# POSTECH-CVLab/SCNeRF

Measured on AMD Instinct MI355X. Metric: rays/sec (64+128 samples/ray) train-step, higher is better.
Workload: dtype f32 (3 x fp16 MFMA products per product, fp32 accumulate); 1 GPU; configs[1]: 4096 rays x (64 coarse + 128 fine), coarse+fine NeRF (D=8, W=256), fwd+bwd of render_rays per GPU, perturb=1, raw_noise_std=1; precomputed rays of a fixed camera; rays_per_gpu=4096, parallelism=ray-parallel x1, no collective at N = 1

## Files before the change

include/scnerf_hip.h:

```cpp
#ifndef SCNERF_HIP_H
#define SCNERF_HIP_H

#include <stdint.h>

#ifdef __cplusplus
extern "C" {
#endif

#define SCNERF_ABI_VERSION 4

int scnerf_abi_version(void);


int scnerf_searchsorted(const float* a, const float* v, int64_t* out, int nrow, int nrow_a,
                        int nrow_v, int na, int nv, int side_left, void* stream);

int scnerf_sample_pdf(const float* bins, const float* weights, const float* u, int u_row_stride,
                      float* samples, int64_t* inds, float* cdf, int n, int nb, int ns,
                      void* stream);

int scnerf_render_randoms(unsigned long long seed, unsigned long long call, float* t_rand, long long n_t_rand,
                          float* u, long long n_u, float* noise_c, long long n_noise_c, float* noise_f,
                          long long n_noise_f, float raw_noise_std, void* stream);

// ... 327 lines not shown

int scnerf_ray_expand(const int* slot_of, long long n, long long n_live, int s_tot, int s_fine, const float* rgb_l,
                      const float* disp_l, const float* acc_l, const float* depth_l, const float* z_std_l, const float* raw_l,
                      const float* z_vals_l, const float* z_samples_l, const float* rgb0, const float* disp0,
                      const float* acc0, const float* depth0, float* rgb_map, float* disp_map, float* acc_map,
                      float* depth_map, float* z_std, float* raw, float* z_vals, float* z_samples, void* stream);


long long scnerf_live_compact_workspace_ints(long long n_samples);
int scnerf_live_compact(const float* d_raw, long long n_samples, int* workspace, int* live_idx, unsigned* xoff,
                        float* d_raw_live, int* n_live_dev, int* n_live_host, void* stream);
int scnerf_live_gather(const int* live_idx, long long n_live, long long n_samples, const unsigned* masks, const float* pts,
                       int pt_dims, const float* viewdirs, int vd_stride, int samples_per_ray, unsigned* masks_live,
                       float* pts_live, float* vd_live, void* stream);
int scnerf_live_scatter_rows(const float* src, const int* live_idx, float* dst, long long n_live, int w, long long n,
                             void* stream);
int scnerf_live_remap_maxima(const int* live_idx, long long n_live, const float* amax_src, int n_chunks_src,
                             long long chunk_src, float* amax_dst, int n_chunks_dst, long long chunk_dst, int rows, void* stream);
int scnerf_mlp_bwd_h3_masks(int pt_dims, const float* d_raw, const float* pts, const float* viewdirs, int vd_stride,
                            int samples_per_ray, const float* wpacked_bwd, const short* stream_bwd, const float* scales,
                            const unsigned* masks, float* grads, float* d_pts, float* d_views, long long n_samples,
                            float* chunk_amax, int n_chunks, long long chunk_samples, int* guard_flags, int* guard_any,
                            float* guard_report, int lean, void* stream);
int scnerf_nerf_wgrad_h3_live(int pt_dims, const float* save, long long n_samples_src, int n_chunks_src,
                              const float* grads_live, const float* d_raw, const int* live_idx, const unsigned* xoff,
                              long long n_live, int n_chunks_live, float* workspace, float* flat_grad, int accumulate,
                              const float* amax_x_live, const float* amax_z_live, const float* scales, const float* flat_params,
                              void* ev_before, void* ev_after, void* stream);


long long scnerf_occ_compact_workspace_ints(long long n_samples);
int scnerf_occ_compact(const float* pts, long long n_samples, const float* viewdirs, int vd_stride, int samples_per_ray,
                       const int* bits, int R, float lo_x, float lo_y, float lo_z, float inv_x, float inv_y, float inv_z,
                       int* workspace, int* live_idx, int* slot_of, float* pts_live, float* vd_live, int* n_live_dev,
                       int* n_live_host, void* stream);
int scnerf_occ_expand_raw(const float* raw_live, const int* slot_of, float* raw, long long n_samples, long long n_live,
                          void* stream);
int scnerf_occ_probe_points(long long first_cell, long long n_cells, int R, int k, float lo_x, float lo_y, float lo_z,
                            float cell_x, float cell_y, float cell_z, float off0, float off1, float off2, float* pts,
                            void* stream);
int scnerf_occ_accumulate(const float* raw, float sigma_min, long long first_cell, long long n_cells, int R, int k, int* bits,
                          void* stream);
int scnerf_occ_dilate(const int* bits_in, int* bits_out, int R, void* stream);

long long scnerf_occ_compact4_workspace_ints(long long n_samples);
int scnerf_occ_compact4(const float* pts, long long n_samples, const float* viewdirs, int vd_stride, int samples_per_ray,
// ... 24 lines not shown
```

scnerf_amd/_capi.py:

```python
from __future__ import annotations

import ctypes
import os
from ctypes import c_int, c_longlong, c_void_p, c_float, c_double

D = c_double

F = c_float

_HERE = os.path.dirname(os.path.abspath(__file__))
LIB_PATH = os.environ.get("SCNERF_HIP_LIB") or os.path.join(_HERE, "libscnerf_hip.so")

P = c_void_p
I = c_int
LL = c_longlong

PROTOTYPES = {
    "scnerf_abi_version": [],
    "scnerf_searchsorted": [P, P, P, I, I, I, I, I, I, P],
    "scnerf_sample_pdf": [P, P, P, I, P, P, P, I, I, I, P],
    "scnerf_render_randoms": [ctypes.c_ulonglong, ctypes.c_ulonglong, P, LL, P, LL, P, LL, P, LL, F, P],
    "scnerf_coarse_sample": [P, I, P, P, P, P, I, I, I, P],
    "scnerf_fine_sample": [P, I, P, P, P, I, P, P, P, P, P, P, I, I, I, P],
    "scnerf_camera_rays_fwd": [P, P, I, P, I, P, P, F, I, P, P, F, I, P, F, P, F, I, I, I, I, P, P, I, P],
# ... 62 lines not shown
    "scnerf_nerf_wgrad_h3": [I, P, P, P, LL, I, P, P, I, P, P, P, P, P, P],
    "scnerf_wgrad256_half": [P, P, LL, I, P, P, P, P, P, P],
    "scnerf_wgrad_half_narrow": [P, I, P, I, I, I, LL, I, P, P, P, P, P, I, LL, P],
    "scnerf_mlp_fwd_h3_lean": [I, P, P, I, I, P, P, P, P, P, LL, P, I, LL, P, P, P, I, P],
    "scnerf_mlp_bwd_h3_lean": [I, P, P, P, I, I, P, P, P, P, P, P, P, LL, P, I, LL, P, P, P, I, P],
    "scnerf_coarse_stage_fwd_h3_lean": [P, I, P, P, I, P, P, P, P, P, I, P, P, P, P, P, P, P, P, I, I, P, I, LL,
                                        P, P, P, I, P],
    "scnerf_fine_stage_fwd_h3_lean": [P, I, P, P, P, I, P, P, P, P, P, I, P, P, P, P, P, P, P, P, P, P, P, P, I, I, I, P,
                                      I, LL, P, P, P, I, P],
    "scnerf_nerf_wgrad_h3_lean": [I, P, P, P, LL, I, P, P, I, P, P, P, P, P, P, P],
    "scnerf_wgrad_lean_finish": [P, P, P, P, I, P],
    "scnerf_wgrad_lean_finish_pd": [I, P, P, P, P, I, P],
    "scnerf_image_metrics": [P, LL, LL, LL, LL, P, LL, LL, LL, LL, I, I, I, I, P, I, F, F, F, I, P, P, P, P, P],
    "scnerf_ray_batch": [I, ctypes.c_ulonglong, ctypes.c_ulonglong, P, I, I, I, LL, LL, P, I, I, LL, LL, LL, LL, LL, I, I, I,
                         P, P, P, P, P],
    "scnerf_ray_compact": [P, F, P, P, P, P, LL, P],
    "scnerf_ray_rows_gather": [P, P, P, LL, I, LL, P],
    "scnerf_ray_expand": [P, LL, LL, I, I] + [P] * 8 + [P] * 4 + [P] * 8 + [P],
    "scnerf_live_compact": [P, LL, P, P, P, P, P, P, P],
    "scnerf_live_gather": [P, LL, LL, P, P, I, P, I, I, P, P, P, P],
    "scnerf_live_remap_maxima": [P, LL, P, I, LL, P, I, LL, I, P],
    "scnerf_live_scatter_rows": [P, P, P, LL, I, LL, P],
    "scnerf_mlp_bwd_h3_masks": [I, P, P, P, I, I, P, P, P, P, P, P, P, LL, P, I, LL, P, P, P, I, P],
    "scnerf_nerf_wgrad_h3_live": [I, P, LL, I, P, P, P, P, LL, I, P, P, I, P, P, P, P, P, P, P],
    "scnerf_occ_compact": [P, LL, P, I, I, P, I, F, F, F, F, F, F, P, P, P, P, P, P, P, P],
    "scnerf_occ_expand_raw": [P, P, P, LL, LL, P],
    "scnerf_occ_probe_points": [LL, LL, I, I, F, F, F, F, F, F, F, F, F, P, P],
    "scnerf_occ_accumulate": [P, F, LL, LL, I, I, P, P],
    "scnerf_occ_dilate": [P, P, I, P],
    "scnerf_occ_compact4": [P, LL, P, I, I, P, I, F, F, F, F, F, F, P, P, P, P, P, P, P, P],
    "scnerf_occ_probe_points_inverted": [LL, LL, I, I, F, F, F, F, F, F, F, F, F, P, P],
    "scnerf_seg_compact": [P, LL, I, I, I, P, P, I, P, I, F, F, F, F, F, F, P, P, P, P, P, P, P, P],
    "scnerf_seg_expand_raw": [P, P, P, LL, I, I, I, LL, P],
    "scnerf_seg_transmittance": [P, P, P, I, LL, I, I, I, I, I, D, P, P, P, P],
}


SIZE_FUNCS = {"scnerf_mlp_save_floats": [I, LL], "scnerf_mlp_grad_floats": [LL],
              "scnerf_wgrad_workspace_floats": [I, I, I],
              "scnerf_nerf_wgrad_workspace_floats": [I],
              "scnerf_h3_scale_floats": [],
              "scnerf_wgrad_chunk_samples": [LL, I],
              "scnerf_camera_bwd_workspace_floats": [I],
              "scnerf_live_compact_workspace_ints": [LL],
              "scnerf_occ_compact_workspace_ints": [LL],
              "scnerf_occ_compact4_workspace_ints": [LL],
# ... 50 lines not shown
```

scnerf_amd/csrc/mlp_bwd_h3.hip:

```cpp
#include <cstdint>

#include <scn_wave.h>

#include "launch.h"
#include "mlp_bwd_h3_api.h"
#include "mlp_common.h"
#include "scnerf_hip.h"

extern "C" int scnerf_mlp_bwd_h3_lean(int pt_dims, const float* d_raw, const float* pts, const float* viewdirs,
                                      int vd_stride, int samples_per_ray, const float* wpacked_bwd, const short* stream_bwd,
                                      const float* scales, const float* save, float* grads, float* d_pts, float* d_views,
                                      long long n_samples, float* chunk_amax, int n_chunks, long long chunk_samples,
                                      int* guard_flags, int* guard_any, float* guard_report, int lean, void* stream) {
    SCN_RETURN_IF(!d_raw || !pts || !viewdirs || !wpacked_bwd || !stream_bwd || !scales || !save || !grads, SCN_EINVAL);
    SCN_RETURN_IF(!d_pts != !d_views, SCN_EINVAL);
    SCN_RETURN_IF(samples_per_ray < 1 || vd_stride < 3 || n_samples < 0 || (pt_dims != 3 && pt_dims != 4), SCN_EINVAL);
    SCN_RETURN_IF(n_samples >= (1LL << 31), SCN_ENOSUP);
    SCN_RETURN_IF(chunk_amax && (n_chunks < 1 || chunk_samples < 32 || chunk_samples % 32), SCN_EINVAL);
    SCN_RETURN_IF(!guard_flags != !guard_any || (guard_report && !guard_flags), SCN_EINVAL);
    if (n_samples == 0) return 0;
    hipStream_t st = (hipStream_t)stream;
    const scn::h3b::ChunkMaxima cm{chunk_amax, n_chunks, lean != 0, (long)chunk_samples, {guard_flags, guard_any, guard_report}};
    return pt_dims == 3 ? scn::h3b::bwd_h3_pd3(d_raw, pts, viewdirs, vd_stride, samples_per_ray, wpacked_bwd, stream_bwd, scales, save, grads, d_pts, d_views, n_samples, cm, st)
                        : scn::h3b::bwd_h3_pd4(d_raw, pts, viewdirs, vd_stride, samples_per_ray, wpacked_bwd, stream_bwd, scales, save, grads, d_pts, d_views, n_samples, cm, st);
}

extern "C" int scnerf_mlp_bwd_h3_masks(int pt_dims, const float* d_raw, const float* pts, const float* viewdirs,
                                       int vd_stride, int samples_per_ray, const float* wpacked_bwd, const short* stream_bwd,
                                       const float* scales, const unsigned* masks, float* grads, float* d_pts, float* d_views,
                                       long long n_samples, float* chunk_amax, int n_chunks, long long chunk_samples,
                                       int* guard_flags, int* guard_any, float* guard_report, int lean, void* stream) {
    SCN_RETURN_IF(!masks || n_samples < 0 || (pt_dims != 3 && pt_dims != 4), SCN_EINVAL);
    const long long per_sample = pt_dims == 3 ? scn::mlp::Var<3>::kSavePerSample : scn::mlp::Var<4>::kSavePerSample;
    const uintptr_t base = reinterpret_cast<uintptr_t>(masks) - (uintptr_t)(per_sample * scn::mlp::padded_samples((long)n_samples)) * sizeof(float);
    return scnerf_mlp_bwd_h3_lean(pt_dims, d_raw, pts, viewdirs, vd_stride, samples_per_ray, wpacked_bwd, stream_bwd, scales,
                                  reinterpret_cast<const float*>(base), grads, d_pts, d_views, n_samples, chunk_amax, n_chunks,
                                  chunk_samples, guard_flags, guard_any, guard_report, lean, stream);
}

extern "C" int scnerf_mlp_bwd_h3_guarded(int pt_dims, const float* d_raw, const float* pts, const float* viewdirs,
                                         int vd_stride, int samples_per_ray, const float* wpacked_bwd, const short* stream_bwd,
                                         const float* scales, const float* save, float* grads, float* d_pts, float* d_views,
                                         long long n_samples, float* chunk_amax, int n_chunks, long long chunk_samples,
                                         int* guard_flags, int* guard_any, float* guard_report, void* stream) {
    return scnerf_mlp_bwd_h3_lean(pt_dims, d_raw, pts, viewdirs, vd_stride, samples_per_ray, wpacked_bwd, stream_bwd, scales, save,
                                  grads, d_pts, d_views, n_samples, chunk_amax, n_chunks, chunk_samples, guard_flags, guard_any,
                                  guard_report, 0, stream);
}

extern "C" int scnerf_mlp_bwd_h3(int pt_dims, const float* d_raw, const float* pts, const float* viewdirs, int vd_stride,
                                 int samples_per_ray, const float* wpacked_bwd, const short* stream_bwd, const float* scales,
                                 const float* save, float* grads, float* d_pts, float* d_views, long long n_samples,
                                 float* chunk_amax, int n_chunks, long long chunk_samples, void* stream) {
    return scnerf_mlp_bwd_h3_guarded(pt_dims, d_raw, pts, viewdirs, vd_stride, samples_per_ray, wpacked_bwd, stream_bwd, scales,
                                     save, grads, d_pts, d_views, n_samples, chunk_amax, n_chunks, chunk_samples, nullptr,
                                     nullptr, nullptr, stream);
}
```

scnerf_amd/csrc/mlp_bwd_h3_api.h:

```cpp
#pragma once
#include <hip/hip_runtime.h>

#include "resident_guard.h"

namespace scn {
namespace h3b {

struct ChunkMaxima { float* amax; int n_chunks; int lean; long chunk; ResidentGuard guard; };

int bwd_h3_pd3(const float* d_raw, const float* pts, const float* viewdirs, int vd_stride, int samples_per_ray,
               const float* wpacked_bwd, const short* stream_bwd, const float* scales, const float* save, float* grads,
               float* d_pts, float* d_views, long long n_samples, ChunkMaxima cm, hipStream_t st);
int bwd_h3_pd4(const float* d_raw, const float* pts, const float* viewdirs, int vd_stride, int samples_per_ray,
               const float* wpacked_bwd, const short* stream_bwd, const float* scales, const float* save, float* grads,
               float* d_pts, float* d_views, long long n_samples, ChunkMaxima cm, hipStream_t st);

}
}
```

scnerf_amd/csrc/mlp_bwd_h3_kernel.h:

```cpp
#pragma once
#include <scn_wave.h>

#include "launch.h"
#include "mlp_bwd_h3_api.h"
#include "mlp_h3.h"

namespace scn {
namespace h3b {

using namespace scn::mlp;
using namespace scn::h3;


template <int PD, int L, int NS>
__device__ __forceinline__ void pe_backward(float x, float y, float z, float w, int h, const float (&de)[NS], float* d_a, float* d_b) {
    const float a = h ? y : x;
    float freq = 1.f;
    if constexpr (PD == 3) {
        float ga = de[3 * L];
        float gz = h ? 0.f : de[3 * L + 1];
#pragma unroll
        for (int f = 0; f < L; ++f) {
            float s0, c0, s1, c1;
            sincos(a * freq, &s0, &c0);
// ... 76 lines not shown
            ol[sl][c0] = pack_f16(residual_f16<0>(v[0], s_next, hp), residual_f16<1>(v[1], s_next, hp));
        } else if constexpr (SUB == 8) {
            hp = pack_f16_scaled(v[2], v[3], s_next);
        } else if constexpr (SUB == 9) {
            oh[sl][c0 + 1] = hp;
            ol[sl][c0 + 1] = pack_f16(residual_f16<0>(v[2], s_next, hp), residual_f16<1>(v[3], s_next, hp));
        } else if constexpr (SUB == 10) {
            if constexpr (lab::kNoStore) {
            } else if constexpr (KIND == 2) {
                store_written_through_window(uniform_global_rw(save + (4 * T + q) * 1024), pinned_here(lane16), f32x4{v[0], v[1], v[2], v[3]}, this->window);
            } else {
                store_written_through_at(uniform_global_rw(save + (4 * T + q) * 1024), pinned_here(lane16), f32x4{v[0], v[1], v[2], v[3]});
            }
        }
    }
};


template <int PD>
__host__ __device__ constexpr unsigned bwd_lds_bytes() {
    return (unsigned)(kStreamLds + 256 * 4 + Var<PD>::kES * kThreads * 4);
}

template <int PD, bool IG>
__global__ __launch_bounds__(kThreads, 1) void mlp_bwd_h3_kernel(
    const float* __restrict__ d_raw, const float* __restrict__ pts, const float* __restrict__ viewdirs, int vd_stride,
    int samples_per_ray, const float* __restrict__ wbk, const short* __restrict__ wh3, const float* __restrict__ sc,
    const float* __restrict__ save, float* __restrict__ grads, float* __restrict__ d_pts, float* __restrict__ d_views, long P,
    ChunkMaxima cm) {
    using V = Var<PD>;
    constexpr int ES = V::kES, ET = V::kET;
    claim_whole_register_file();
    const int lane = lane_id();
    const int m = lane & 31, h = lane >> 5;
    const long wave_tile = (long)blockIdx.x * 4 + uniform(wave_id());
    const long p = wave_tile * kSamplesPerWave + m;
    const bool live = p < P;
    const long pc = live ? p : P - 1;
    const long Ppad = padded_samples(P);

    Wave w;
    w.lds = dynamic_lds<char>();
    w.tid16 = threadIdx.x * 16u;
    w.lane16 = (unsigned)lane * 16u;
    float* const alpha_tab = reinterpret_cast<float*>(w.lds + kStreamLds);
    f32x4* const park = reinterpret_cast<f32x4*>(w.lds + kStreamLds + 256 * 4) + threadIdx.x;
    stream_prime(w.ws, wh3, w.lds, w.tid16);
    alpha_tab[threadIdx.x] = wbk[V::kBwdAlphaW + threadIdx.x];

    f32x4 dr = *reinterpret_cast<const f32x4*>(d_raw + pc * 4);
    if (!live) dr = f32x4{0.f, 0.f, 0.f, 0.f};
    const float dsigma = dr[3];

    u32x4 bh[2][16], bl[2][16];
    f32x16 acc[2][2];
    auto section = [&](int offset, int width) {
        return uniform_global_rw(grads + (long)offset * Ppad + wave_tile * (32L * width));
    };
    auto load_gate = [&](int sect) {
        const unsigned* base = reinterpret_cast<const unsigned*>(save + (long)V::kSavePerSample * Ppad);
        return load_at<u32x4>(uniform_global(base + ((long)sect * (Ppad / 32) + wave_tile) * 256), w.lane16);
    };
    auto scale_of = [&](int layer, int what) { return sc[layer * kScaleStride + what]; };
    auto amax_of = [&](float a) { return fmaxf(a, shfl_xor(a, 32)); };
    const int chunk_of_tile = cm.amax ? uniform((int)((unsigned)(wave_tile * kSamplesPerWave) / (unsigned)cm.chunk)) : 0;
    auto note_chunk_max = [&](int job, float v) __attribute__((always_inline)) {
        if (cm.amax == nullptr) return;
        v = fmaxf(v, shfl_xor(v, 16)); v = fmaxf(v, shfl_xor(v, 8)); v = fmaxf(v, shfl_xor(v, 4));
        v = fmaxf(v, shfl_xor(v, 2)); v = fmaxf(v, shfl_xor(v, 1));
        if (lane_id() == 0) atomic_max_nonneg(cm.amax + (long)job * cm.n_chunks + chunk_of_tile, v);
    };
    auto guard = [&](int guard_layer, float am, float s) __attribute__((always_inline)) {
        guard_check(cm.guard, guard_layer, am, s, live, wave_tile);
    };
    using GateEpi = BwdEpi<0>;
    auto make_gate = [&](int layer, float s_in, int mask_sect, int out_offset, int out_width) {
        GateEpi e;
        e.os = inv_pow2(s_in) * scale_of(layer, kSwInv);
        e.s_next = 1.f;
        e.am = 0.f;
        e.save = section(out_offset, out_width);
        e.lane16 = w.lane16;
        e.gate = load_gate(mask_sect);
        return e;
// ... 7 lines not shown
        cut8(x8, s_rgb, rh, rl);
    }
    GateEpi epiv = make_gate(kLayerRgb, s_rgb, 8, kGradDzv, 128);
    epiv.s_next = scale_for(scale_of(kLayerRgb, kBoundAT) * am_rgb);
    block_sync();
    ring_prime(w);
    {
        auto operand = [&](auto, u32x4& xh, u32x4& xl) { xh = rh; xl = rl; };
        tile_pair<0, 1>(w, acc[0], operand, NoFill{});
        tile_pair<1, 1>(w, acc[1], operand, NoFill{});
        epi_all<GateEpi, 0>(epiv, acc[0], bh[1], bl[1]);
        epi_all<GateEpi, 1>(epiv, acc[1], bh[1], bl[1]);
    }
    const float am_v = amax_of(epiv.am);
    note_chunk_max(8, am_v);
    guard(kLayerViews, am_v, epiv.s_next);

    auto hv_operand = [&](auto s_tag, u32x4& xh, u32x4& xl) {
        constexpr int s = decltype(s_tag)::value;
        xh = bh[1][s]; xl = bl[1][s];
    };
    if constexpr (!IG) {
        skip_units<2, 4>(w, NoFill{});
        const long ray = (long)((unsigned)pc / (unsigned)samples_per_ray);
        note_chunk_max(11, fmaxf(fmaxf(1.f, fabsf(viewdirs[ray * vd_stride + 0])),
                                 fmaxf(fabsf(viewdirs[ray * vd_stride + 1]), fabsf(viewdirs[ray * vd_stride + 2]))));
    } else {
        f32x16 acce[2];
        tile_single<2, 4>(w, acce, hv_operand, NoFill{});
        const float os = inv_pow2(epiv.s_next) * scale_of(kLayerViews, kSwInv);
        float dev[16];
#pragma unroll
        for (int r = 0; r < 16; ++r) dev[r] = (acce[0][r] + acce[1][r]) * os;
        const long ray = (long)((unsigned)pc / (unsigned)samples_per_ray);
        note_chunk_max(11, fmaxf(fmaxf(1.f, fabsf(viewdirs[ray * vd_stride + 0])),
                                 fmaxf(fabsf(viewdirs[ray * vd_stride + 1]), fabsf(viewdirs[ray * vd_stride + 2]))));
        float gxy, gz;
        pe_backward<3, 4, 16>(viewdirs[ray * vd_stride + 0], viewdirs[ray * vd_stride + 1], viewdirs[ray * vd_stride + 2], 0.f, h, dev, &gxy, &gz);
        const float oxy = shfl_xor(gxy, 32), oz = shfl_xor(gz, 32);
        if (live && h == 0) {
            d_views[p * 3 + 0] = gxy;
            d_views[p * 3 + 1] = oxy;
            d_views[p * 3 + 2] = gz + oz;
        }
    }
    using LinEpi = BwdEpi<2>;
    LinEpi epif;
    epif.os = inv_pow2(epiv.s_next) * scale_of(kLayerViews, kSwInv);
    epif.s_next = scale_for(scale_of(kLayerViews, kBoundAT) * am_v);
    epif.am = 0.f;
    epif.save = section(kGradDfeat, 256);
    epif.lane16 = w.lane16;
    epif.window = cm.lean ? kStoreWindowShut : kStoreWindowOpen;
    tile_pair<6, 8>(w, acc[0], hv_operand, NoFill{});
    tile_pair<14, 8>(w, acc[1], hv_operand, [&](auto sg) { epi_slot<LinEpi, 0, decltype(sg)::value, 6>(epif, acc[0], bh[0], bl[0]); });
    tile_pair<22, 8>(w, acc[0], hv_operand, [&](auto sg) { epi_slot<LinEpi, 1, decltype(sg)::value, 6>(epif, acc[1], bh[0], bl[0]); });
    tile_pair<30, 8>(w, acc[1], hv_operand, [&](auto sg) { epi_slot<LinEpi, 2, decltype(sg)::value, 6>(epif, acc[0], bh[0], bl[0]); });

    auto trunk_layer = [&](auto x_tag, auto& pend, auto& cur, float bound_a, float bound_extra, int job)
                           __attribute__((always_inline)) {
        constexpr int X = decltype(x_tag)::value;
        auto operand = [&](auto s_tag, u32x4& xh, u32x4& xl) {
            constexpr int s = decltype(s_tag)::value;
            xh = bh[X][s]; xl = bl[X][s];
        };
        using Pend = std::remove_reference_t<decltype(pend)>;
// ... 56 lines not shown
        const float am5 = amax_of(prev.am);
        note_chunk_max(4, am5);
        guard(5, am5, prev.s_next);
        cur.s_next = scale_for(scale_of(5, kBoundAT) * am5);
        constexpr int U0 = 6;
        tile_pair<U0, 16>(w, acc[0], operand, NoFill{});
        tile_pair<U0 + 16, 16>(w, acc[1], operand, [&](auto sg) { epi_slot<GateEpi, 0, decltype(sg)::value, 12>(cur, acc[0], bh[0], bl[0]); });
        tile_pair<U0 + 32, 16>(w, acc[0], operand, [&](auto sg) { epi_slot<GateEpi, 1, decltype(sg)::value, 12>(cur, acc[1], bh[0], bl[0]); });
        tile_pair<U0 + 48, 16>(w, acc[1], operand, [&](auto sg) { epi_slot<GateEpi, 2, decltype(sg)::value, 12>(cur, acc[0], bh[0], bl[0]); });
        prev = cur;
    }
#pragma unroll 1
    for (int l = 4; l >= 2; l -= 2) {
        GateEpi cur = make_gate(l, prev.s_next, l - 1, kGradDz + (l - 1) * 256, 256);
        trunk_layer(I<0>{}, prev, cur, scale_of(l, kBoundAT), 0.f, l - 1);
        GateEpi cur2 = make_gate(l - 1, cur.s_next, l - 2, kGradDz + (l - 2) * 256, 256);
        trunk_layer(I<1>{}, cur, cur2, scale_of(l - 1, kBoundAT), 0.f, l - 2);
        prev = cur2;
    }
    if constexpr (!IG) {
        epi_all<GateEpi, 3>(prev, acc[1], bh[0], bl[0]);
        note_chunk_max(9, amax_of(prev.am));
        guard(0, amax_of(prev.am), prev.s_next);
        float am_e = fmaxf(fmaxf(1.f, fabsf(pts[pc * PD + 0])), fmaxf(fabsf(pts[pc * PD + 1]), fabsf(pts[pc * PD + 2])));
        if constexpr (PD == 4) am_e = fmaxf(am_e, fabsf(pts[pc * PD + 3]));
        note_chunk_max(10, am_e);
    } else {
        auto operand = [&](auto s_tag, u32x4& xh, u32x4& xl) {
            constexpr int s = decltype(s_tag)::value;
            xh = bh[0][s]; xl = bl[0][s];
        };
        float de[ES];
        tile_pair<6, 16>(w, acc[0], operand, [&](auto sg) { epi_slot<GateEpi, 3, decltype(sg)::value, 9>(prev, acc[1], bh[0], bl[0]); });
        const float os0 = inv_pow2(prev.s_next) * scale_of(0, kSwInv);
        note_chunk_max(9, amax_of(prev.am));
        guard(0, amax_of(prev.am), prev.s_next);
        auto add_pair = [&](auto t0_tag, f32x16 (&a)[2]) {
            constexpr int T0 = decltype(t0_tag)::value;
#pragma unroll
            for (int x = 0; x < 2; ++x)
                if (16 * (T0 + x) < ES) {
#pragma unroll
                    for (int q = 0; q < 4; ++q) {
                        const f32x4 pk = park[(4 * (T0 + x) + q) * kThreads];
#pragma unroll
                        for (int j = 0; j < 4; ++j) de[16 * (T0 + x) + 4 * q + j] = __builtin_fmaf(a[x][4 * q + j], os0, pk[j]);
                    }
                }
        };
        add_pair(I<0>{}, acc[0]);
        if constexpr (ET == 4) {
            tile_pair<22, 16>(w, acc[1], operand, NoFill{});
            add_pair(I<2>{}, acc[1]);
        }
        float ga, gb;
        {
            float am_e = fmaxf(fmaxf(1.f, fabsf(pts[pc * PD + 0])), fmaxf(fabsf(pts[pc * PD + 1]), fabsf(pts[pc * PD + 2])));
            if constexpr (PD == 4) am_e = fmaxf(am_e, fabsf(pts[pc * PD + 3]));
            note_chunk_max(10, am_e);
        }
        pe_backward<PD, 10, ES>(pts[pc * PD + 0], pts[pc * PD + 1], pts[pc * PD + 2], PD == 4 ? pts[pc * PD + (PD - 1)] : 0.f, h, de, &ga, &gb);
        const float oa = shfl_xor(ga, 32), ob = shfl_xor(gb, 32);
        if (live && h == 0) {
            d_pts[p * PD + 0] = ga;
            d_pts[p * PD + 1] = oa;
            if constexpr (PD == 3) {
                d_pts[p * PD + 2] = gb + ob;
            } else {
                d_pts[p * PD + 2] = gb;
                d_pts[p * PD + (PD - 1)] = ob;
            }
        }
    }
}


template <int PD, bool IG>
inline int launch_bwd_h3_as(const float* d_raw, const float* pts, const float* viewdirs, int vd_stride, int samples_per_ray,
                            const float* wpacked_bwd, const short* stream_bwd, const float* scales, const float* save,
                            float* grads, float* d_pts, float* d_views, long long n_samples, ChunkMaxima cm, hipStream_t st) {
    constexpr unsigned lds = bwd_lds_bytes<PD>();
    SCN_LDS_OPT_IN((mlp_bwd_h3_kernel<PD, IG>), lds);
    hipLaunchKernelGGL((mlp_bwd_h3_kernel<PD, IG>), dim3(scn_ceil_div(n_samples, kSamplesPerBlock)), dim3(kThreads), lds, st,
                       d_raw, pts, viewdirs, vd_stride, samples_per_ray, wpacked_bwd, stream_bwd, scales, save, grads, d_pts,
                       d_views, (long)n_samples, cm);
    return scn_launch_status();
}

template <int PD>
inline int launch_bwd_h3(const float* d_raw, const float* pts, const float* viewdirs, int vd_stride, int samples_per_ray,
                         const float* wpacked_bwd, const short* stream_bwd, const float* scales, const float* save,
                         float* grads, float* d_pts, float* d_views, long long n_samples, ChunkMaxima cm, hipStream_t st) {
    return d_pts ? launch_bwd_h3_as<PD, true>(d_raw, pts, viewdirs, vd_stride, samples_per_ray, wpacked_bwd, stream_bwd, scales,
                                              save, grads, d_pts, d_views, n_samples, cm, st)
                 : launch_bwd_h3_as<PD, false>(d_raw, pts, viewdirs, vd_stride, samples_per_ray, wpacked_bwd, stream_bwd, scales,
                                               save, grads, nullptr, nullptr, n_samples, cm, st);
}


}
}
```

scnerf_amd/functional.py:

```python
from __future__ import annotations

from dataclasses import dataclass
from typing import Optional

import torch

from . import mlp_layout as ML
from . import ops

Tensor = torch.Tensor


@dataclass
class RenderConfig:
    n_samples: int
    n_importance: int
    lindisp: bool
    white_bkgd: bool
    track: bool = True


_host_cache = {}


# ... 159 lines not shown
            live = (rgb_f, disp_f, acc_f, depth_f, z_std, raw_f, z_f, z_s)
        rgb, disp, acc, depth, z_std, raw, z_vals, z_samples = ops.ray_expand(slot_of, n_live, live, coarse, tot, sf)
        return rgb, disp, acc, depth, raw, z_std, z_vals, z_samples

    @staticmethod
    def _stage_composite_bwd(stage, rays, white_bkgd, g_rgb, g_disp, g_acc, g_depth, g_raw, want, live):
        z, _, raw, noise, _, _ = stage
        d_raw, d_rd = ops.composite_bwd(raw, z, rays, noise, white_bkgd, _c(g_rgb), _c(g_disp), _c(g_acc),
                                        _c(g_depth), _c(g_raw), want_d_rays_d=want)
        return d_raw, d_rd, ops.live_compact(d_raw) if live else None

    @staticmethod
    def _stage_dgrad(stage, first, rays, spr, wbk, d_rays, accumulate, planes=None, guard=None, lean=False, flat_params=None,
                     guard_fwd=None):
        z, pts, raw, noise, save, maxima = stage
        d_raw, d_rd, L = first
        want = d_rays is not None
        P = z.shape[0] * spr
        if L is not None and L.n > 0 and ops.live_guard_tripped(guard_fwd):
            L = None
        if L is not None and L.n > ops.LIVE_MAX_SHARE * P:
            L = None
        if L is not None and L.n > 0:
            masks, pts_l, vd_l = ops.live_gather(L, save, pts, rays[:, 8:11], spr)
            maxima_l = ops.live_maxima(L, maxima)
            guard_l = ops.live_guard_record(guard, L.n) if guard is not None else None
            grads, d_pts, d_views = ops.mlp_bwd_live(L, masks, pts_l, vd_l, wbk, planes, maxima_l, input_grad=want, lean=lean,
                                                     guard=guard_l)
            if guard_l is not None and guard_l.rerun and ops.live_guard_tripped(guard_l):
                L = None
            else:
                if guard_l is not None:
                    ops.live_guard_keep(guard_l)
                maxima = maxima_l
                if want:
                    d_pts, d_views = ops.live_scatter_rows(L, d_pts), ops.live_scatter_rows(L, d_views)
        if L is None:
            grads, d_pts, d_views = ops.mlp_bwd(d_raw, pts, rays[:, 8:11], spr, wbk, save, planes=planes, maxima=maxima,
                                                input_grad=want, guard=guard, lean=lean)
        elif L.n == 0:
            grads = maxima = None
            d_pts, d_views = (torch.zeros((P, 3), dtype=torch.float32, device=rays.device) for _ in range(2)) if want else (None, None)
        if want:
            ops.ray_reduce(d_pts, d_views, z, d_rd, d_rays, accumulate)
        return save, grads, d_raw, P, maxima, lean, flat_params, L

    @staticmethod
    def _stage_wgrad(pending, into=None):
        save, grads, d_raw, P, maxima, lean, flat_params, L = pending
        if L is not None:
            if L.n == 0:
                return None if into is not None else torch.zeros(ML.N_PARAMS, dtype=torch.float32, device=d_raw.device)
            out = ops.nerf_wgrad_live(L, save, grads, d_raw, maxima, flat_grad=into, accumulate=into is not None, lean=lean,
                                      flat_params=flat_params)
            return None if into is not None else out
        if into is not None:
            ops.nerf_wgrad(save, grads, d_raw, P, flat_grad=into, accumulate=True, maxima=maxima, lean=lean,
                           flat_params=flat_params)
# ... 86 lines not shown
```

scnerf_amd/ops.py:

```python
from __future__ import annotations

import os
from typing import Optional

import numpy as np
import torch

from . import _capi
from . import mlp_layout as ML

Tensor = torch.Tensor


class _Profile:

    def __init__(self):
        self.enabled = False
        self.records = {}

    def reset(self, enabled=False):
        self.records = {}
        self.enabled = enabled

    class _Region:
# ... 1380 lines not shown
    lay = ML.layout(pd)
    Pp, Pl = ML.padded_samples(L.P), ML.padded_samples(L.n)
    if save.numel() < lay.save_floats(L.P):
        raise ValueError("activation workspace too small")
    masks = save[lay.save_floats_per_sample * Pp:]
    dev = pts.device
    masks_l = torch.empty(ML.MASK_WORDS_PER_SAMPLE * Pl, dtype=torch.int32, device=dev)
    pts_l = torch.empty((L.n, pd), dtype=torch.float32, device=dev)
    vd_l = torch.empty((L.n, 3), dtype=torch.float32, device=dev)
    st = _capi.load().scnerf_live_gather(_p(L.idx), L.n, L.P, _p(masks), _p(pts), pd, vptr, vstride, int(samples_per_ray),
                                         _p(masks_l), _p(pts_l), _p(vd_l), _stream())
    _capi.check(st, "scnerf_live_gather")
    return masks_l, pts_l, vd_l


def live_maxima(L: LiveSamples, maxima: ChunkMaxima) -> ChunkMaxima:
    out = ChunkMaxima(L.n, maxima.x.device)
    st = _capi.load().scnerf_live_remap_maxima(_p(L.idx), L.n, _p(maxima.x), maxima.chunks, maxima.chunk_samples, _p(out.x),
                                               out.chunks, out.chunk_samples, 8, _stream())
    _capi.check(st, "scnerf_live_remap_maxima")
    return out


def mlp_bwd_live(L: LiveSamples, masks: Tensor, pts: Tensor, viewdirs: Tensor, wpacked_bwd: Tensor, rw: ResidentWeights,
                 maxima: ChunkMaxima, input_grad: bool = True, lean: bool = False, guard: Optional[GuardRecord] = None):
    pd = rw.pd
    n, dev = L.n, pts.device
    _f(pts, "pts"), _f(viewdirs, "viewdirs"), _f(wpacked_bwd, "wpacked_bwd")
    if pts.numel() != n * pd or viewdirs.numel() != n * 3 or masks.numel() != ML.MASK_WORDS_PER_SAMPLE * ML.padded_samples(n):
        raise ValueError("not the compact batch of this compaction")
    if wpacked_bwd.numel() != ML.layout(pd).bwd_total:
        raise ValueError("wpacked_bwd has the wrong size")
    grads = torch.empty(ML.grad_floats(n), dtype=torch.float32, device=dev)
    d_pts = torch.empty((n, pd), dtype=torch.float32, device=dev) if input_grad else None
    d_views = torch.empty((n, 3), dtype=torch.float32, device=dev) if input_grad else None
    with PROFILE.region("mlp_bwd_h3_kernel%s/P=%d live" % ("" if pd == 3 else "/pd4", n), 2 * _MAC_PER_SAMPLE[pd] * n):
        maxima.scales = rw.scales
        st = _capi.load().scnerf_mlp_bwd_h3_masks(
            pd, _p(L.d_raw), _p(pts), _p(viewdirs), 3, 1, _p(wpacked_bwd), _p(rw.bwd), _p(rw.scales), _p(masks), _p(grads),
            _p(d_pts), _p(d_views), n, _p(maxima.z), maxima.chunks, maxima.chunk_samples, *_guard_args(guard), int(lean),
            _stream())
    _capi.check(st, "scnerf_mlp_bwd_h3_masks")
    if guard is not None and guard.mode == "strict":
        _GUARD_LAST[guard.name] = guard
        guard.raise_if_tripped()
    return grads, d_pts, d_views


def live_scatter_rows(L: LiveSamples, rows: Tensor) -> Tensor:
    _f(rows, "rows")
    w = rows.shape[1]
    out = torch.empty((L.P, w), dtype=torch.float32, device=rows.device)
    st = _capi.load().scnerf_live_scatter_rows(_p(rows), _p(L.idx), _p(out), L.n, w, L.P, _stream())
    _capi.check(st, "scnerf_live_scatter_rows")
    return out


def nerf_wgrad_live(L: LiveSamples, save: Tensor, grads: Tensor, d_raw: Tensor, maxima: ChunkMaxima,
                    flat_grad: Optional[Tensor] = None, pd: int = 3, accumulate: bool = False, lean: bool = False,
                    flat_params: Optional[Tensor] = None) -> Tensor:
    lib = _capi.load()
    chunks_src, chunks = wgrad_chunks(L.P), wgrad_chunks(L.n)
    key = (chunks_src, str(save.device))
    if key not in _wgrad_ws:
        _wgrad_ws[key] = torch.empty(lib.scnerf_nerf_wgrad_workspace_floats(chunks_src), dtype=torch.float32, device=save.device)
# ... 356 lines not shown
```

Measured before the change: 398,200 rays/s.

## Index live samples directly in MLP backward instead of gathering gates and inputs

Adds a gather-mode variant of the h3 backward kernel that reads gate masks, points and view directions of live samples through the live index from the full-size saved buffers. It also writes d_pts and d_views straight into dense rows. This removes the separate live_gather and live_scatter_rows launches and their intermediate buffers, and it is on by default via a new switch. In exchange, gate loads become per-lane scattered accesses instead of contiguous tile loads, and the dense gradient outputs must be zero-filled over all samples.

```diff
diff --git a/include/scnerf_hip.h b/include/scnerf_hip.h
--- a/include/scnerf_hip.h
+++ b/include/scnerf_hip.h
@@ -373,6 +373,11 @@
                             const unsigned* masks, float* grads, float* d_pts, float* d_views, long long n_samples,
                             float* chunk_amax, int n_chunks, long long chunk_samples, int* guard_flags, int* guard_any,
                             float* guard_report, int lean, void* stream);
+int scnerf_mlp_bwd_h3_live(int pt_dims, const float* d_raw_live, const int* live_idx, long long n_live, const float* save,
+                           long long n_samples_src, int samples_per_ray_src, const float* pts, const float* viewdirs,
+                           int vd_stride, const float* wpacked_bwd, const short* stream_bwd, const float* scales, float* grads,
+                           float* d_pts, float* d_views, float* chunk_amax, int n_chunks, long long chunk_samples,
+                           int* guard_flags, int* guard_any, float* guard_report, int lean, void* stream);
 int scnerf_nerf_wgrad_h3_live(int pt_dims, const float* save, long long n_samples_src, int n_chunks_src,
                               const float* grads_live, const float* d_raw, const int* live_idx, const unsigned* xoff,
                               long long n_live, int n_chunks_live, float* workspace, float* flat_grad, int accumulate,
diff --git a/scnerf_amd/_capi.py b/scnerf_amd/_capi.py
--- a/scnerf_amd/_capi.py
+++ b/scnerf_amd/_capi.py
@@ -108,6 +108,7 @@
     "scnerf_live_remap_maxima": [P, LL, P, I, LL, P, I, LL, I, P],
     "scnerf_live_scatter_rows": [P, P, P, LL, I, LL, P],
     "scnerf_mlp_bwd_h3_masks": [I, P, P, P, I, I, P, P, P, P, P, P, P, LL, P, I, LL, P, P, P, I, P],
+    "scnerf_mlp_bwd_h3_live": [I, P, P, LL, P, LL, I, P, P, I, P, P, P, P, P, P, P, I, LL, P, P, P, I, P],
     "scnerf_nerf_wgrad_h3_live": [I, P, LL, I, P, P, P, P, LL, I, P, P, I, P, P, P, P, P, P, P],
     "scnerf_occ_compact": [P, LL, P, I, I, P, I, F, F, F, F, F, F, P, P, P, P, P, P, P, P],
     "scnerf_occ_expand_raw": [P, P, P, LL, LL, P],
diff --git a/scnerf_amd/csrc/mlp_bwd_h3.hip b/scnerf_amd/csrc/mlp_bwd_h3.hip
--- a/scnerf_amd/csrc/mlp_bwd_h3.hip
+++ b/scnerf_amd/csrc/mlp_bwd_h3.hip
@@ -38,6 +38,29 @@
                                   chunk_samples, guard_flags, guard_any, guard_report, lean, stream);
 }
 
+extern "C" int scnerf_mlp_bwd_h3_live(int pt_dims, const float* d_raw_live, const int* live_idx, long long n_live,
+                                      const float* save, long long n_samples_src, int samples_per_ray_src, const float* pts,
+                                      const float* viewdirs, int vd_stride, const float* wpacked_bwd, const short* stream_bwd,
+                                      const float* scales, float* grads, float* d_pts, float* d_views, float* chunk_amax,
+                                      int n_chunks, long long chunk_samples, int* guard_flags, int* guard_any,
+                                      float* guard_report, int lean, void* stream) {
+    SCN_RETURN_IF(pt_dims != 3 && pt_dims != 4, SCN_EINVAL);
+    SCN_RETURN_IF(pt_dims != 3, SCN_ENOSUP);
+    SCN_RETURN_IF(n_live < 0 || n_samples_src < 1 || n_live > n_samples_src, SCN_EINVAL);
+    SCN_RETURN_IF(n_samples_src > (1LL << 22) - 128, SCN_ENOSUP);
+    SCN_RETURN_IF(!d_raw_live || !live_idx || !pts || !viewdirs || !wpacked_bwd || !stream_bwd || !scales || !save || !grads,
+                  SCN_EINVAL);
+    SCN_RETURN_IF(!d_pts != !d_views, SCN_EINVAL);
+    SCN_RETURN_IF(samples_per_ray_src < 1 || vd_stride < 3, SCN_EINVAL);
+    SCN_RETURN_IF(chunk_amax && (n_chunks < 1 || chunk_samples < 32 || chunk_samples % 32), SCN_EINVAL);
+    SCN_RETURN_IF(!guard_flags != !guard_any || (guard_report && !guard_flags), SCN_EINVAL);
+    if (n_live == 0) return 0;
+    const scn::h3b::ChunkMaxima cm{chunk_amax, n_chunks, lean != 0, (long)chunk_samples, {guard_flags, guard_any, guard_report}};
+    return scn::h3b::bwd_h3_pd3_live(d_raw_live, pts, viewdirs, vd_stride, samples_per_ray_src, wpacked_bwd, stream_bwd, scales, save,
+                                     grads, d_pts, d_views, n_live, cm, scn::h3b::LiveGates{live_idx, (long)n_samples_src},
+                                     (hipStream_t)stream);
+}
+
 extern "C" int scnerf_mlp_bwd_h3_guarded(int pt_dims, const float* d_raw, const float* pts, const float* viewdirs,
                                          int vd_stride, int samples_per_ray, const float* wpacked_bwd, const short* stream_bwd,
                                          const float* scales, const float* save, float* grads, float* d_pts, float* d_views,
diff --git a/scnerf_amd/csrc/mlp_bwd_h3_api.h b/scnerf_amd/csrc/mlp_bwd_h3_api.h
--- a/scnerf_amd/csrc/mlp_bwd_h3_api.h
+++ b/scnerf_amd/csrc/mlp_bwd_h3_api.h
@@ -8,6 +8,8 @@
 
 struct ChunkMaxima { float* amax; int n_chunks; int lean; long chunk; ResidentGuard guard; };
 
+struct LiveGates { const int* live_idx; long n_src; };
+
 int bwd_h3_pd3(const float* d_raw, const float* pts, const float* viewdirs, int vd_stride, int samples_per_ray,
                const float* wpacked_bwd, const short* stream_bwd, const float* scales, const float* save, float* grads,
                float* d_pts, float* d_views, long long n_samples, ChunkMaxima cm, hipStream_t st);
@@ -15,5 +17,9 @@
                const float* wpacked_bwd, const short* stream_bwd, const float* scales, const float* save, float* grads,
                float* d_pts, float* d_views, long long n_samples, ChunkMaxima cm, hipStream_t st);
 
+int bwd_h3_pd3_live(const float* d_raw, const float* pts, const float* viewdirs, int vd_stride, int samples_per_ray,
+                    const float* wpacked_bwd, const short* stream_bwd, const float* scales, const float* save, float* grads,
+                    float* d_pts, float* d_views, long long n_live, ChunkMaxima cm, LiveGates lg, hipStream_t st);
+
 }
 }
diff --git a/scnerf_amd/csrc/mlp_bwd_h3_kernel.h b/scnerf_amd/csrc/mlp_bwd_h3_kernel.h
--- a/scnerf_amd/csrc/mlp_bwd_h3_kernel.h
+++ b/scnerf_amd/csrc/mlp_bwd_h3_kernel.h
@@ -122,12 +122,12 @@
     return (unsigned)(kStreamLds + 256 * 4 + Var<PD>::kES * kThreads * 4);
 }
 
-template <int PD, bool IG>
+template <int PD, bool IG, bool GATHER = false>
 __global__ __launch_bounds__(kThreads, 1) void mlp_bwd_h3_kernel(
     const float* __restrict__ d_raw, const float* __restrict__ pts, const float* __restrict__ viewdirs, int vd_stride,
     int samples_per_ray, const float* __restrict__ wbk, const short* __restrict__ wh3, const float* __restrict__ sc,
     const float* __restrict__ save, float* __restrict__ grads, float* __restrict__ d_pts, float* __restrict__ d_views, long P,
-    ChunkMaxima cm) {
+    ChunkMaxima cm, LiveGates lg) {
     using V = Var<PD>;
     constexpr int ES = V::kES, ET = V::kET;
     claim_whole_register_file();
@@ -151,6 +151,15 @@
     f32x4 dr = *reinterpret_cast<const f32x4*>(d_raw + pc * 4);
     if (!live) dr = f32x4{0.f, 0.f, 0.f, 0.f};
     const float dsigma = dr[3];
+    unsigned goff = 0u;
+    if constexpr (GATHER) {
+        unsigned d = (unsigned)lg.live_idx[pc];
+        if (d >= (unsigned)lg.n_src) d = (unsigned)lg.n_src - 1u;
+        goff = (d >> 5) * 1024u + (((unsigned)h << 5) | (d & 31u)) * 16u;
+    }
+    auto dense_row = [&]() -> long { return (long)((goff >> 10) * 32u + ((goff >> 4) & 31u)); };
+    auto src_row = [&]() -> long { if constexpr (GATHER) return dense_row(); else return pc; };
+    auto dst_row = [&]() -> long { if constexpr (GATHER) return dense_row(); else return p; };
 
     u32x4 bh[2][16], bl[2][16];
     f32x16 acc[2][2];
@@ -158,8 +167,14 @@
         return uniform_global_rw(grads + (long)offset * Ppad + wave_tile * (32L * width));
     };
     auto load_gate = [&](int sect) {
-        const unsigned* base = reinterpret_cast<const unsigned*>(save + (long)V::kSavePerSample * Ppad);
-        return load_at<u32x4>(uniform_global(base + ((long)sect * (Ppad / 32) + wave_tile) * 256), w.lane16);
+        if constexpr (GATHER) {
+            const long Ppad_src = padded_samples(lg.n_src);
+            const unsigned* base = reinterpret_cast<const unsigned*>(save + (long)V::kSavePerSample * Ppad_src);
+            return load_at<u32x4>(uniform_global(base + (long)sect * (Ppad_src / 32) * 256), goff);
+        } else {
+            const unsigned* base = reinterpret_cast<const unsigned*>(save + (long)V::kSavePerSample * Ppad);
+            return load_at<u32x4>(uniform_global(base + ((long)sect * (Ppad / 32) + wave_tile) * 256), w.lane16);
+        }
     };
     auto scale_of = [&](int layer, int what) { return sc[layer * kScaleStride + what]; };
     auto amax_of = [&](float a) { return fmaxf(a, shfl_xor(a, 32)); };
@@ -213,7 +228,7 @@
     };
     if constexpr (!IG) {
         skip_units<2, 4>(w, NoFill{});
-        const long ray = (long)((unsigned)pc / (unsigned)samples_per_ray);
+        const long ray = (long)((unsigned)src_row() / (unsigned)samples_per_ray);
         note_chunk_max(11, fmaxf(fmaxf(1.f, fabsf(viewdirs[ray * vd_stride + 0])),
                                  fmaxf(fabsf(viewdirs[ray * vd_stride + 1]), fabsf(viewdirs[ray * vd_stride + 2]))));
     } else {
@@ -223,16 +238,17 @@
         float dev[16];
 #pragma unroll
         for (int r = 0; r < 16; ++r) dev[r] = (acce[0][r] + acce[1][r]) * os;
-        const long ray = (long)((unsigned)pc / (unsigned)samples_per_ray);
+        const long ray = (long)((unsigned)src_row() / (unsigned)samples_per_ray);
         note_chunk_max(11, fmaxf(fmaxf(1.f, fabsf(viewdirs[ray * vd_stride + 0])),
                                  fmaxf(fabsf(viewdirs[ray * vd_stride + 1]), fabsf(viewdirs[ray * vd_stride + 2]))));
         float gxy, gz;
         pe_backward<3, 4, 16>(viewdirs[ray * vd_stride + 0], viewdirs[ray * vd_stride + 1], viewdirs[ray * vd_stride + 2], 0.f, h, dev, &gxy, &gz);
         const float oxy = shfl_xor(gxy, 32), oz = shfl_xor(gz, 32);
         if (live && h == 0) {
-            d_views[p * 3 + 0] = gxy;
-            d_views[p * 3 + 1] = oxy;
-            d_views[p * 3 + 2] = gz + oz;
+            const long pr = dst_row();
+            d_views[pr * 3 + 0] = gxy;
+            d_views[pr * 3 + 1] = oxy;
+            d_views[pr * 3 + 2] = gz + oz;
         }
     }
     using LinEpi = BwdEpi<2>;
@@ -335,8 +351,9 @@
         epi_all<GateEpi, 3>(prev, acc[1], bh[0], bl[0]);
         note_chunk_max(9, amax_of(prev.am));
         guard(0, amax_of(prev.am), prev.s_next);
-        float am_e = fmaxf(fmaxf(1.f, fabsf(pts[pc * PD + 0])), fmaxf(fabsf(pts[pc * PD + 1]), fabsf(pts[pc * PD + 2])));
-        if constexpr (PD == 4) am_e = fmaxf(am_e, fabsf(pts[pc * PD + 3]));
+        const long ps = src_row();
+        float am_e = fmaxf(fmaxf(1.f, fabsf(pts[ps * PD + 0])), fmaxf(fabsf(pts[ps * PD + 1]), fabsf(pts[ps * PD + 2])));
+        if constexpr (PD == 4) am_e = fmaxf(am_e, fabsf(pts[ps * PD + 3]));
         note_chunk_max(10, am_e);
     } else {
         auto operand = [&](auto s_tag, u32x4& xh, u32x4& xl) {
@@ -367,36 +384,39 @@
             add_pair(I<2>{}, acc[1]);
         }
         float ga, gb;
+        const long ps = src_row();
         {
-            float am_e = fmaxf(fmaxf(1.f, fabsf(pts[pc * PD + 0])), fmaxf(fabsf(pts[pc * PD + 1]), fabsf(pts[pc * PD + 2])));
-            if constexpr (PD == 4) am_e = fmaxf(am_e, fabsf(pts[pc * PD + 3]));
+            float am_e = fmaxf(fmaxf(1.f, fabsf(pts[ps * PD + 0])), fmaxf(fabsf(pts[ps * PD + 1]), fabsf(pts[ps * PD + 2])));
+            if constexpr (PD == 4) am_e = fmaxf(am_e, fabsf(pts[ps * PD + 3]));
             note_chunk_max(10, am_e);
         }
-        pe_backward<PD, 10, ES>(pts[pc * PD + 0], pts[pc * PD + 1], pts[pc * PD + 2], PD == 4 ? pts[pc * PD + (PD - 1)] : 0.f, h, de, &ga, &gb);
+        pe_backward<PD, 10, ES>(pts[ps * PD + 0], pts[ps * PD + 1], pts[ps * PD + 2], PD == 4 ? pts[ps * PD + (PD - 1)] : 0.f, h, de, &ga, &gb);
         const float oa = shfl_xor(ga, 32), ob = shfl_xor(gb, 32);
         if (live && h == 0) {
-            d_pts[p * PD + 0] = ga;
-            d_pts[p * PD + 1] = oa;
+            const long pr = dst_row();
+            d_pts[pr * PD + 0] = ga;
+            d_pts[pr * PD + 1] = oa;
             if constexpr (PD == 3) {
-                d_pts[p * PD + 2] = gb + ob;
+                d_pts[pr * PD + 2] = gb + ob;
             } else {
-                d_pts[p * PD + 2] = gb;
-                d_pts[p * PD + (PD - 1)] = ob;
-            }
-        }
-    }
-}
-
-
-template <int PD, bool IG>
+                d_pts[pr * PD + 2] = gb;
+                d_pts[pr * PD + (PD - 1)] = ob;
+            }
+        }
+    }
+}
+
+
+template <int PD, bool IG, bool GATHER = false>
 inline int launch_bwd_h3_as(const float* d_raw, const float* pts, const float* viewdirs, int vd_stride, int samples_per_ray,
                             const float* wpacked_bwd, const short* stream_bwd, const float* scales, const float* save,
-                            float* grads, float* d_pts, float* d_views, long long n_samples, ChunkMaxima cm, hipStream_t st) {
+                            float* grads, float* d_pts, float* d_views, long long n_samples, ChunkMaxima cm, hipStream_t st,
+                            LiveGates lg = LiveGates{nullptr, 0}) {
     constexpr unsigned lds = bwd_lds_bytes<PD>();
-    SCN_LDS_OPT_IN((mlp_bwd_h3_kernel<PD, IG>), lds);
-    hipLaunchKernelGGL((mlp_bwd_h3_kernel<PD, IG>), dim3(scn_ceil_div(n_samples, kSamplesPerBlock)), dim3(kThreads), lds, st,
+    SCN_LDS_OPT_IN((mlp_bwd_h3_kernel<PD, IG, GATHER>), lds);
+    hipLaunchKernelGGL((mlp_bwd_h3_kernel<PD, IG, GATHER>), dim3(scn_ceil_div(n_samples, kSamplesPerBlock)), dim3(kThreads), lds, st,
                        d_raw, pts, viewdirs, vd_stride, samples_per_ray, wpacked_bwd, stream_bwd, scales, save, grads, d_pts,
-                       d_views, (long)n_samples, cm);
+                       d_views, (long)n_samples, cm, lg);
     return scn_launch_status();
 }
 
@@ -410,6 +430,17 @@
                                                save, grads, nullptr, nullptr, n_samples, cm, st);
 }
 
-
-}
-}
+template <int PD>
+inline int launch_bwd_h3_live(const float* d_raw, const float* pts, const float* viewdirs, int vd_stride, int samples_per_ray,
+                              const float* wpacked_bwd, const short* stream_bwd, const float* scales, const float* save,
+                              float* grads, float* d_pts, float* d_views, long long n_live, ChunkMaxima cm, LiveGates lg,
+                              hipStream_t st) {
+    return d_pts ? launch_bwd_h3_as<PD, true, true>(d_raw, pts, viewdirs, vd_stride, samples_per_ray, wpacked_bwd, stream_bwd,
+                                                    scales, save, grads, d_pts, d_views, n_live, cm, st, lg)
+                 : launch_bwd_h3_as<PD, false, true>(d_raw, pts, viewdirs, vd_stride, samples_per_ray, wpacked_bwd, stream_bwd,
+                                                     scales, save, grads, nullptr, nullptr, n_live, cm, st, lg);
+}
+
+
+}
+}
diff --git a/scnerf_amd/csrc/mlp_bwd_h3_pd3_live.hip b/scnerf_amd/csrc/mlp_bwd_h3_pd3_live.hip
--- /dev/null
+++ b/scnerf_amd/csrc/mlp_bwd_h3_pd3_live.hip
@@ -0,0 +1,14 @@
+#include "mlp_bwd_h3_kernel.h"
+
+namespace scn {
+namespace h3b {
+
+int bwd_h3_pd3_live(const float* d_raw, const float* pts, const float* viewdirs, int vd_stride, int samples_per_ray,
+                    const float* wpacked_bwd, const short* stream_bwd, const float* scales, const float* save, float* grads,
+                    float* d_pts, float* d_views, long long n_live, ChunkMaxima cm, LiveGates lg, hipStream_t st) {
+    return launch_bwd_h3_live<3>(d_raw, pts, viewdirs, vd_stride, samples_per_ray, wpacked_bwd, stream_bwd, scales, save, grads,
+                                 d_pts, d_views, n_live, cm, lg, st);
+}
+
+}
+}
diff --git a/scnerf_amd/functional.py b/scnerf_amd/functional.py
--- a/scnerf_amd/functional.py
+++ b/scnerf_amd/functional.py
@@ -205,18 +205,24 @@
         if L is not None and L.n > ops.LIVE_MAX_SHARE * P:
             L = None
         if L is not None and L.n > 0:
-            masks, pts_l, vd_l = ops.live_gather(L, save, pts, rays[:, 8:11], spr)
+            index = ops.live_gates() == "index"
+            if not index:
+                masks, pts_l, vd_l = ops.live_gather(L, save, pts, rays[:, 8:11], spr)
             maxima_l = ops.live_maxima(L, maxima)
             guard_l = ops.live_guard_record(guard, L.n) if guard is not None else None
-            grads, d_pts, d_views = ops.mlp_bwd_live(L, masks, pts_l, vd_l, wbk, planes, maxima_l, input_grad=want, lean=lean,
-                                                     guard=guard_l)
+            if index:
+                grads, d_pts, d_views = ops.mlp_bwd_live(L, save, pts, rays[:, 8:11], wbk, planes, maxima_l, input_grad=want,
+                                                         lean=lean, guard=guard_l, samples_per_ray=spr)
+            else:
+                grads, d_pts, d_views = ops.mlp_bwd_live(L, masks, pts_l, vd_l, wbk, planes, maxima_l, input_grad=want,
+                                                         lean=lean, guard=guard_l)
             if guard_l is not None and guard_l.rerun and ops.live_guard_tripped(guard_l):
                 L = None
             else:
                 if guard_l is not None:
                     ops.live_guard_keep(guard_l)
                 maxima = maxima_l
-                if want:
+                if want and not index:
                     d_pts, d_views = ops.live_scatter_rows(L, d_pts), ops.live_scatter_rows(L, d_views)
         if L is None:
             grads, d_pts, d_views = ops.mlp_bwd(d_raw, pts, rays[:, 8:11], spr, wbk, save, planes=planes, maxima=maxima,
diff --git a/scnerf_amd/ops.py b/scnerf_amd/ops.py
--- a/scnerf_amd/ops.py
+++ b/scnerf_amd/ops.py
@@ -1426,25 +1426,49 @@
     return out
 
 
+LIVE_GATES = ("index", "gather")
+_LIVE_GATES = _Switch(LIVE_GATES, "SCNERF_LIVE_GATES", "index", "live_gates is one of " + ", ".join(LIVE_GATES))
+
+
+def live_gates(mode: Optional[str] = None) -> str:
+    return _LIVE_GATES(mode)
+
+
 def mlp_bwd_live(L: LiveSamples, masks: Tensor, pts: Tensor, viewdirs: Tensor, wpacked_bwd: Tensor, rw: ResidentWeights,
-                 maxima: ChunkMaxima, input_grad: bool = True, lean: bool = False, guard: Optional[GuardRecord] = None):
+                 maxima: ChunkMaxima, input_grad: bool = True, lean: bool = False, guard: Optional[GuardRecord] = None,
+                 samples_per_ray: Optional[int] = None):
     pd = rw.pd
     n, dev = L.n, pts.device
-    _f(pts, "pts"), _f(viewdirs, "viewdirs"), _f(wpacked_bwd, "wpacked_bwd")
-    if pts.numel() != n * pd or viewdirs.numel() != n * 3 or masks.numel() != ML.MASK_WORDS_PER_SAMPLE * ML.padded_samples(n):
-        raise ValueError("not the compact batch of this compaction")
-    if wpacked_bwd.numel() != ML.layout(pd).bwd_total:
-        raise ValueError("wpacked_bwd has the wrong size")
     grads = torch.empty(ML.grad_floats(n), dtype=torch.float32, device=dev)
-    d_pts = torch.empty((n, pd), dtype=torch.float32, device=dev) if input_grad else None
-    d_views = torch.empty((n, 3), dtype=torch.float32, device=dev) if input_grad else None
-    with PROFILE.region("mlp_bwd_h3_kernel%s/P=%d live" % ("" if pd == 3 else "/pd4", n), 2 * _MAC_PER_SAMPLE[pd] * n):
-        maxima.scales = rw.scales
-        st = _capi.load().scnerf_mlp_bwd_h3_masks(
-            pd, _p(L.d_raw), _p(pts), _p(viewdirs), 3, 1, _p(wpacked_bwd), _p(rw.bwd), _p(rw.scales), _p(masks), _p(grads),
-            _p(d_pts), _p(d_views), n, _p(maxima.z), maxima.chunks, maxima.chunk_samples, *_guard_args(guard), int(lean),
-            _stream())
-    _capi.check(st, "scnerf_mlp_bwd_h3_masks")
+    tag = "mlp_bwd_h3_kernel%s/P=%d live" % ("" if pd == 3 else "/pd4", n)
+    if samples_per_ray is not None:
+        vptr, vstride, lay, P = _network_args(pts, viewdirs, wpacked_bwd, "bwd", pd, masks)
+        if pd != 3 or P != L.P or masks.numel() < lay.save_floats(P):
+            raise ValueError("not the pass of this compaction")
+        d_pts = torch.zeros((P, 3), dtype=torch.float32, device=dev) if input_grad else None
+        d_views = torch.zeros((P, 3), dtype=torch.float32, device=dev) if input_grad else None
+        with PROFILE.region(tag, 2 * _MAC_PER_SAMPLE[pd] * n):
+            maxima.scales = rw.scales
+            st = _capi.load().scnerf_mlp_bwd_h3_live(
+                pd, _p(L.d_raw), _p(L.idx), n, _p(masks), P, int(samples_per_ray), _p(pts), vptr, vstride, _p(wpacked_bwd),
+                _p(rw.bwd), _p(rw.scales), _p(grads), _p(d_pts), _p(d_views), _p(maxima.z), maxima.chunks,
+                maxima.chunk_samples, *_guard_args(guard), int(lean), _stream())
+        _capi.check(st, "scnerf_mlp_bwd_h3_live")
+    else:
+        _f(pts, "pts"), _f(viewdirs, "viewdirs"), _f(wpacked_bwd, "wpacked_bwd")
+        if pts.numel() != n * pd or viewdirs.numel() != n * 3 or masks.numel() != ML.MASK_WORDS_PER_SAMPLE * ML.padded_samples(n):
+            raise ValueError("not the compact batch of this compaction")
+        if wpacked_bwd.numel() != ML.layout(pd).bwd_total:
+            raise ValueError("wpacked_bwd has the wrong size")
+        d_pts = torch.empty((n, pd), dtype=torch.float32, device=dev) if input_grad else None
+        d_views = torch.empty((n, 3), dtype=torch.float32, device=dev) if input_grad else None
+        with PROFILE.region(tag, 2 * _MAC_PER_SAMPLE[pd] * n):
+            maxima.scales = rw.scales
+            st = _capi.load().scnerf_mlp_bwd_h3_masks(
+                pd, _p(L.d_raw), _p(pts), _p(viewdirs), 3, 1, _p(wpacked_bwd), _p(rw.bwd), _p(rw.scales), _p(masks), _p(grads),
+                _p(d_pts), _p(d_views), n, _p(maxima.z), maxima.chunks, maxima.chunk_samples, *_guard_args(guard), int(lean),
+                _stream())
+        _capi.check(st, "scnerf_mlp_bwd_h3_masks")
     if guard is not None and guard.mode == "strict":
         _GUARD_LAST[guard.name] = guard
         guard.raise_if_tripped()
```

Result: slower. 352,800 rays/s (-11.4%).
